# paLeziart/quadruped-reactive-walking

Hardware: AMD Instinct MI355X
Metric: control-steps/sec (MPC+WBC) (higher is better)
Workload: dtype f64

## Files before the change

### quadruped-reactive-walking_amd/csrc/chain_sweep.h

```cpp
#pragma once
#include <hip/hip_runtime.h>

#include "qrw_device.h"

namespace qrw {

constexpr int kCol = 14;
constexpr int kSlot = 168;
__host__ __device__ constexpr int chain_gap(int m) { return 0; }
__host__ __device__ constexpr int chain_slot(int slot, int m) { return slot * kSlot + (slot >= m ? chain_gap(m) : 0); }
__device__ __forceinline__ int chain_row_t(int lane) {
  const int l = lane & 15;
  return (l < 12) ? l : 11;
}
__host__ __device__ constexpr int chain_lds_doubles(int slots, int m) { return slots * kSlot + chain_gap(m); }

__device__ __forceinline__ double dpp_step12(double r, double x, const double (&m)[12]) {
  double a0 = r;
  asm("s_nop 1\n\t"
      "v_fmac_f64_dpp %0, %1, %2 row_newbcast:0 row_mask:0xf bank_mask:0xf\n\t"
      "v_fmac_f64_dpp %0, %1, %3 row_newbcast:1 row_mask:0xf bank_mask:0xf\n\t"
      "v_fmac_f64_dpp %0, %1, %4 row_newbcast:2 row_mask:0xf bank_mask:0xf\n\t"
      "v_fmac_f64_dpp %0, %1, %5 row_newbcast:3 row_mask:0xf bank_mask:0xf\n\t"
      "v_fmac_f64_dpp %0, %1, %6 row_newbcast:4 row_mask:0xf bank_mask:0xf\n\t"
// ... 28 lines not shown
  int lo = __double2loint(v), hi = __double2hiint(v);
  asm("s_nop 1\n\tv_permlane16_swap_b32 %0, %0\n\tv_permlane16_swap_b32 %1, %1" : "+v"(lo), "+v"(hi));
  return __hiloint2double(hi, lo);
}

template <int NC>
__device__ __forceinline__ void chain_forward_paired(const double* sN, double* sX, double* sDump, int lane) {
  constexpr int N = NC, m = N >> 1, LA = m, LB = N - 1 - m, NP = LA / 2;
  static_assert(LA % 2 == 0 && LB == LA - 1, "paired sweeps need an even chain length");
  const int i = ((lane & 15) < 12) ? (lane & 15) : 11;
  const int h = lane >> 5;
  const bool rw = (lane & 16) != 0;
  const bool own = (lane & 15) < 12;
  const double* pm = sN + (rw ? m * kSlot + chain_gap(m) : 0) + h * kSlot + i;
  double* px = sX + (rw ? (m + 1) * 12 : 0) + i;
  const double* pr = px + h * 12;
  double* dump = sDump + i;
  double* ps_odd = (own && h == 1) ? px : dump;
  double* ps_even = (own && h == 0) ? px : dump;
  double* ps_oddA = (own && h == 1 && !rw) ? px : dump;
  double x = px[0], pB = 0.0;
  ChainOp b0, b1;
  auto fetch = [&](ChainOp& b, int p) {
    const double* q = pm + 2 * p * kSlot;
#pragma unroll
    for (int c = 0; c < 12; c++) b.m[c] = __hip_atomic_load(q + c * kCol, __ATOMIC_RELAXED, __HIP_MEMORY_SCOPE_WAVEFRONT);
    b.r = pr[(2 * p + 1) * 12];
  };
  auto pair = [&](const ChainOp& b, int p) {
    const int t1 = 2 * p + 1, t2 = t1 + 1;
    x = dpp_step12(b.r, x, b.m);
    x = swap_halves(x);
    if (t1 == LB) pB = x;
    (t1 < LB ? ps_odd : ps_oddA)[t1 * 12] = x;
    x = dpp_step12(b.r, x, b.m);
    if (t2 < LA) {
      x = swap_halves(x);
      ps_even[t2 * 12] = x;
    }
  };
  fetch(b0, 0);
#pragma unroll
  for (int p = 0; p < NP; p += 2) {
    if (p + 1 < NP) fetch(b1, p + 1);
    __builtin_amdgcn_sched_barrier(0);
    pair(b0, p);
    if (p + 1 < NP) {
      if (p + 2 < NP) fetch(b0, p + 2);
      __builtin_amdgcn_sched_barrier(0);
      pair(b1, p + 1);
    }
  }
  x += swap_rows16(pB);
  if (lane >= 32 && lane < 44) sX[m * 12 + i] = x;
}
template <int NC>
__device__ __forceinline__ void chain_backward_paired(const double* sN, double* sX, double* sDump, int lane) {
  constexpr int N = NC, m = N >> 1, LA = m, LB = N - 1 - m, NP = LA / 2;
  static_assert(LA % 2 == 0 && LB == LA - 1, "paired sweeps need an even chain length");
  const int i = ((lane & 15) < 12) ? (lane & 15) : 11;
  const int h = lane >> 5;
  const bool rw = (lane & 16) != 0;
  const bool own = (lane & 15) < 12;
  const int ib = chain_row_t(lane);
  const double* pm = sN + ((rw ? (N - 1) : m) - LA - h) * kSlot + (rw ? chain_gap(m) : 0) + ib * kCol;
  double* px = sX + ((rw ? N : m) - LA) * 12 + i;
  const double* pr = px - h * 12;
  double* dump = sDump + i;
  double* ps_odd = (own && h == 1) ? px : dump;
  double* ps_even = (own && h == 0) ? px : dump;
  double* ps_lastA = (own && h == 1 && !rw) ? px : dump;
  double x = sX[m * 12 + i];
  ChainOp b0, b1;
  auto fetch = [&](ChainOp& b, int p) {
    const qrw_d2* q = reinterpret_cast<const qrw_d2*>(pm + (LA - 2 * p - 1) * kSlot);
#pragma unroll
    for (int c = 0; c < 6; c++) {
      const qrw_d2 v = q[c];
      b.m[2 * c] = v.x;
      b.m[2 * c + 1] = v.y;
    }
    b.r = pr[(LA - 2 * p - 1) * 12];
  };
  auto pair = [&](const ChainOp& b, int p) {
    const int t1 = 2 * p + 1, t2 = t1 + 1;
    x = dpp_step12(b.r, x, b.m);
    x = swap_halves(x);
    ps_odd[(LA - t1) * 12] = x;
    x = dpp_step12(b.r, x, b.m);
    if (t2 < LA) {
      x = swap_halves(x);
      ps_even[(LA - t2) * 12] = x;
    } else {
      ps_lastA[(LA - t2) * 12] = x;
    }
  };
  fetch(b0, 0);
#pragma unroll
  for (int p = 0; p < NP; p += 2) {
    if (p + 1 < NP) fetch(b1, p + 1);
    __builtin_amdgcn_sched_barrier(0);
    pair(b0, p);
    if (p + 1 < NP) {
      if (p + 2 < NP) fetch(b0, p + 2);
      __builtin_amdgcn_sched_barrier(0);
      pair(b1, p + 1);
    }
  }
}

template <int NC>
__device__ __forceinline__ void chain_forward_quad(const double* sN, double* sX, double* sDump, int lane) {
  constexpr int N = NC, m = N >> 1, LA = m, LB = N - 1 - m, NQ = LA / 4;
  static_assert(LA % 4 == 0 && LB == LA - 1, "the 2 + 2 half order needs a chain length that is a multiple of 4");
  const int i = ((lane & 15) < 12) ? (lane & 15) : 11;
  const int h = lane >> 5;
  const bool rw = (lane & 16) != 0;
  const bool own = (lane & 15) < 12;
  const double* pm = sN + (rw ? m * kSlot + chain_gap(m) : 0) + 2 * h * kSlot + i;
  double* px = sX + (rw ? (m + 1) * 12 : 0) + i;
  const double* pr = px + 2 * h * 12;
  double* dump = sDump + i;
  double* ps_lo = (own && h == 0) ? px : dump;
  double* ps_hi = (own && h == 1) ? px : dump;
  double* ps_hiA = (own && h == 1 && !rw) ? px : dump;
  double x = px[0], pB = 0.0;
  ChainOp bX, bY;
  auto fetch = [&](ChainOp& b, int s) {
    const double* q = pm + s * kSlot;
#pragma unroll
    for (int c = 0; c < 12; c++) b.m[c] = __hip_atomic_load(q + c * kCol, __ATOMIC_RELAXED, __HIP_MEMORY_SCOPE_WAVEFRONT);
    b.r = pr[(s + 1) * 12];
  };
  fetch(bX, 0);
  fetch(bY, 1);
#pragma unroll
  for (int q = 0; q < NQ; q++) {
    const int t = 4 * q;
    __builtin_amdgcn_sched_barrier(0);
    x = dpp_step12(bX.r, x, bX.m);
    ps_lo[(t + 1) * 12] = x;
    x = dpp_step12(bY.r, x, bY.m);
    x = swap_halves(x);
    ps_hi[(t + 2) * 12] = x;
    x = dpp_step12(bX.r, x, bX.m);
    if (t + 3 == LB) pB = x;
    (t + 3 < LB ? ps_hi : ps_hiA)[(t + 3) * 12] = x;
    if (q + 1 < NQ) fetch(bX, t + 4);
    __builtin_amdgcn_sched_barrier(0);
    x = dpp_step12(bY.r, x, bY.m);
    if (q + 1 < NQ) {
      x = swap_halves(x);
      ps_lo[(t + 4) * 12] = x;
      fetch(bY, t + 5);
    }
  }
  x += swap_rows16(pB);
  if (lane >= 32 && lane < 44) sX[m * 12 + i] = x;
}
template <int NC>
__device__ __forceinline__ void chain_backward_quad(const double* sN, double* sX, double* sDump, int lane) {
  constexpr int N = NC, m = N >> 1, LA = m, LB = N - 1 - m, NQ = LA / 4;
  static_assert(LA % 4 == 0 && LB == LA - 1, "the 2 + 2 half order needs a chain length that is a multiple of 4");
  const int i = ((lane & 15) < 12) ? (lane & 15) : 11;
  const int h = lane >> 5;
  const bool rw = (lane & 16) != 0;
  const bool own = (lane & 15) < 12;
  const int ib = chain_row_t(lane);
  const double* pm = sN + ((rw ? (N - 1) : m) - LA - 2 * h) * kSlot + (rw ? chain_gap(m) : 0) + ib * kCol;
  double* px = sX + ((rw ? N : m) - LA) * 12 + i;
  const double* pr = px - 2 * h * 12;
  double* dump = sDump + i;
  double* ps_lo = (own && h == 0) ? px : dump;
  double* ps_hi = (own && h == 1) ? px : dump;
  double* ps_lastA = (own && h == 1 && !rw) ? px : dump;
  double x = sX[m * 12 + i];
  ChainOp bX, bY;
  auto fetch = [&](ChainOp& b, int t) {
    const qrw_d2* q = reinterpret_cast<const qrw_d2*>(pm + (LA - t) * kSlot);
#pragma unroll
    for (int c = 0; c < 6; c++) {
      const qrw_d2 v = q[c];
      b.m[2 * c] = v.x;
      b.m[2 * c + 1] = v.y;
    }
    b.r = pr[(LA - t) * 12];
  };
  fetch(bX, 1);
  fetch(bY, 2);
#pragma unroll
  for (int q = 0; q < NQ; q++) {
    const int t = 4 * q;
    __builtin_amdgcn_sched_barrier(0);
    x = dpp_step12(bX.r, x, bX.m);
    ps_lo[(LA - t - 1) * 12] = x;
    x = dpp_step12(bY.r, x, bY.m);
    x = swap_halves(x);
    ps_hi[(LA - t - 2) * 12] = x;
    x = dpp_step12(bX.r, x, bX.m);
    ps_hi[(LA - t - 3) * 12] = x;
    if (q + 1 < NQ) fetch(bX, t + 5);
    __builtin_amdgcn_sched_barrier(0);
    x = dpp_step12(bY.r, x, bY.m);
    if (q + 1 < NQ) {
      x = swap_halves(x);
      ps_lo[(LA - t - 4) * 12] = x;
      fetch(bY, t + 6);
    } else {
      ps_lastA[0] = x;
    }
  }
// ... 154 lines not shown
```

### quadruped-reactive-walking_amd/csrc/mpc_kernel.hip

```cpp
#include <hip/hip_runtime.h>
#include <math.h>
#include <stdint.h>

#include <type_traits>
#include <vector>

#include "chain_sweep.h"
#include "qrw_device.h"
#include "qrw_kernels.h"

namespace qrw {

namespace {

constexpr int kMatSz = 144;
constexpr int kWSz = 36;

template <int NW>
struct alignas(16) MpcLdsT {
  static constexpr int S = 16 * NW;
  double sN[chain_lds_doubles(S, S / 2)];
  double sX[(S + 2) * 12];
  double sDump[(S / 2 + 2) * 12];
  double sE[S * 12];
  double sW[S * kWSz];
  double sOm[S * 12];
  double sDg[S * 12];
  double sA[kMatSz];
  double sB[kMatSz];
  double sRed[4];
  unsigned long long sBal[2];
  double sPre[8];
};

template <int NW>
__device__ __forceinline__ void wg_sync_t() {
  if constexpr (NW == 1) asm volatile("" ::: "memory");
  else __syncthreads();
}
#define wg_sync() wg_sync_t<NW>()
#ifdef QRW_PROFILE_PHASES
#define PH_DECL unsigned long long ph_t0 = __builtin_amdgcn_s_memtime(), ph_acc[10] = {0,0,0,0,0,0,0,0,0,0};
#ifndef QRW_PH_MASK
#define QRW_PH_MASK 0x3FF
#endif
#define PH(i) do { if ((QRW_PH_MASK >> (i)) & 1) { unsigned long long t_ = __builtin_amdgcn_s_memtime(); ph_acc[i] += t_ - ph_t0; ph_t0 = t_; } } while (0)
#elif defined(QRW_MARK_PHASES)
#define PH_DECL
#define PH(i) asm volatile("; QRW_PHASE " #i)
#else
#define PH_DECL
#define PH(i)
#endif

__device__ __forceinline__ void cone_apply(const double f[3], double mu, double out[5]) {
  out[0] = f[0] - mu * f[2];
  out[1] = -f[0] - mu * f[2];
  out[2] = f[1] - mu * f[2];
  out[3] = -f[1] - mu * f[2];
  out[4] = -f[2];
}
__device__ __forceinline__ void cone_apply_t(const double w[5], double mu, double out[3]) {
  out[0] = w[0] - w[1];
  out[1] = w[2] - w[3];
  out[2] = -mu * (w[0] + w[1] + w[2] + w[3]) - w[4];
}

template <int NW, bool CL = false>
__device__ __forceinline__ void nb_next(const double v[3], double same[3], double shifted[3], double* sE, int k, int j,
                                        int lane, bool has_next) {
  if constexpr (NW == 1) {
    const int s4 = (CL && !has_next) ? lane : lane + 4, s2 = (CL && !has_next) ? lane : lane + 2;
#pragma unroll
    for (int t = 0; t < 3; t++) { same[t] = shfl(v[t], s4); shifted[t] = shfl(v[t], s2); }
  } else {
#pragma unroll
    for (int t = 0; t < 3; t++) sE[k * 12 + 3 * j + t] = v[t];
    __syncthreads();
    const int kn = has_next ? k + 1 : k;
#pragma unroll
    for (int t = 0; t < 3; t++) { same[t] = sE[kn * 12 + 3 * j + t]; shifted[t] = sE[kn * 12 + 3 * ((j + 2) & 3) + t]; }
    __syncthreads();
  }
}
template <int NW, bool CL = false>
__device__ __forceinline__ void nb_prev(const double v[3], double same[3], double shifted[3], double* sE, int k, int j,
                                        int lane, bool has_prev) {
  if constexpr (NW == 1) {
    const int s4 = (CL && !has_prev) ? lane : lane - 4, s2 = (CL && !has_prev) ? lane : lane - 2;
#pragma unroll
    for (int t = 0; t < 3; t++) { same[t] = shfl(v[t], s4); shifted[t] = shfl(v[t], s2); }
  } else {
#pragma unroll
// ... 374 lines not shown
  return task;
}
template <int NW>
__device__ __forceinline__ bool pre_may_park(const MpcArgs& a, unsigned long long* sh, int tid) {
  int ok = 0;
  if (tid == 0) ok = pre_claim(a) ? 1 : 0;
  if constexpr (NW == 1) {
    ok = __builtin_amdgcn_readfirstlane(ok);
  } else {
    int* si = reinterpret_cast<int*>(sh);
    __syncthreads();
    if (tid == 0) si[0] = ok;
    __syncthreads();
    ok = si[0];
    __syncthreads();
  }
  return ok != 0;
}
__device__ __forceinline__ int pre_level(const MpcArgs& a, int iter, int it_resume, double r, double r_prev) {
  if (a.pre_levels < 2 || it_resume == 0) return 0;
  const int nl = a.pre_levels - 1;
  float rem = (float)(4000 - iter);
  if (r_prev > r && r > 1.0) rem = fminf(rem, 200.0f * __logf((float)r) / __logf((float)(r_prev / r)));
  int bin = (int)(rem / (float)a.pre_bin);
  bin = bin < 0 ? 0 : (bin > nl - 1 ? nl - 1 : bin);
  return 1 + (nl - 1 - bin);
}
template <int NW>
__device__ __forceinline__ void pre_end_chunk(const MpcArgs& a, int b, bool parked, int level, int tid) {
  asm volatile("s_waitcnt vmcnt(0)" ::: "memory");
  if constexpr (NW > 1) __syncthreads();
  if (tid == 0) {
    if (parked) {
      __builtin_amdgcn_fence(__ATOMIC_RELEASE, "agent");
      asm volatile("s_waitcnt vmcnt(0)" ::: "memory");
      const unsigned slot = __hip_atomic_fetch_add(&a.pre_ctr[kPreLevelWord + 2 * level + 1], 1u, __ATOMIC_RELAXED, __HIP_MEMORY_SCOPE_AGENT);
      if (slot < (unsigned)a.pre_cap) __hip_atomic_store(&a.pre_queue[(size_t)level * a.pre_cap + slot], b, __ATOMIC_RELAXED, __HIP_MEMORY_SCOPE_AGENT);
      else pre_set_error(a, 2u);
      __hip_atomic_fetch_add(&a.pre_ctr[kPreParks], 1u, __ATOMIC_RELAXED, __HIP_MEMORY_SCOPE_AGENT);
    } else {
      __hip_atomic_fetch_add(&a.pre_ctr[kPreDone], 1u, __ATOMIC_RELAXED, __HIP_MEMORY_SCOPE_AGENT);
    }
    __hip_atomic_fetch_add(&a.pre_ctr[kPreProgress], 1u, __ATOMIC_RELAXED, __HIP_MEMORY_SCOPE_AGENT);
  }
}

template <int NW, bool FULL, bool SEQ, bool PRE = false>
__global__ __launch_bounds__(64 * NW, 1) void mpc_solve_kernel(MpcArgs a) {
  static_assert(!(SEQ && PRE), "one queueing mode at a time");
  __shared__ MpcLdsT<NW> L;
  constexpr int T = 64 * NW;
  PH_DECL
  const int tid = threadIdx.x;
  const int lane = tid & 63, wv = tid >> 6;
#ifdef QRW_DEBUG_POISON
  if constexpr (!SEQ && !PRE) {
    const double qnan = __longlong_as_double(-1ll);
    auto fill = [&](double* p, int n) { for (int e = tid; e < n; e += 64 * NW) p[e] = qnan; };
    switch (a.pre_bin) {
      case 1: fill(L.sN, (int)(sizeof(L.sN) / 8)); break;
      case 2: fill(L.sX, (int)(sizeof(L.sX) / 8)); break;
      case 3: fill(L.sDump, (int)(sizeof(L.sDump) / 8)); break;
      case 4: fill(L.sE, (int)(sizeof(L.sE) / 8)); break;
      case 5: fill(L.sW, (int)(sizeof(L.sW) / 8)); break;
      case 6: fill(L.sOm, (int)(sizeof(L.sOm) / 8)); break;
      case 7: fill(L.sDg, (int)(sizeof(L.sDg) / 8)); break;
      case 8: fill(L.sA, kMatSz); break;
      case 9: fill(L.sB, kMatSz); break;
      case 10: fill(L.sRed, 4); fill(L.sPre, 8); break;
      default: break;
    }
    __syncthreads();
  }
#endif
  {
  int b, seq_s = 0;
#ifdef QRW_SEQ_STATS
  unsigned long long task_t0 = 0;
#endif
  if constexpr (SEQ) {
    const int task = seq_next_task<NW>(a, &L.sBal[0], tid, (int)blockIdx.x < a.seq_groups);
    if (task < 0) return;
#ifdef QRW_SEQ_STATS
    task_t0 = __builtin_amdgcn_s_memrealtime();
#endif
    seq_s = task / a.B;
    b = task - seq_s * a.B;
  } else if constexpr (PRE) {
    if ((int)blockIdx.x + a.pre_block0 < a.B) {
      b = a.order ? a.order[blockIdx.x] : blockIdx.x;
    } else {
      b = pre_next_task<NW>(a, &L.sBal[0], tid);
      if (b < 0) return;
    }
  } else {
    b = a.order ? a.order[blockIdx.x] : blockIdx.x;
  }
  int it_resume = 0;
  bool aborted = false;
  if constexpr (PRE) {
    const int pit = __hip_atomic_load(&a.pause_it[b], __ATOMIC_RELAXED, __HIP_MEMORY_SCOPE_AGENT);
    if ((int)blockIdx.x + a.pre_block0 >= a.B) it_resume = pit;
    else aborted = (pit != 0);
  }
  const bool resumed = PRE && it_resume > 0;
  if constexpr (PRE) { if (tid < 8) L.sPre[tid] = 0.0; }
#ifdef QRW_TRACE_RES
  if (!resumed && a.prof) for (int e = tid; e < kMpcProfItems; e += T) a.prof[(size_t)b * kMpcProfItems + e] = 0.0;
#endif
  const int k = 16 * wv + (lane >> 2), j = lane & 3;
  const int N = a.N;
  const bool act = FULL ? true : (k < N);
  const bool has_next = act && (k + 1 < N);
  const bool has_prev = act && (k > 0);
  const bool next_here = has_next;
  const double mN = next_here ? 1.0 : 0.0, mN6 = (next_here && j >= 2) ? a.dt : 0.0;
  const double mP = has_prev ? 1.0 : 0.0, mP6 = (has_prev && j < 2) ? a.dt : 0.0;
  const double mG = (j >= 2) ? 1.0 : 0.0, mGN = (j >= 2 && next_here) ? 1.0 : 0.0;
  const int kp = has_prev ? k - 1 : k;
  const int kx = act ? chain_pos(k, N >> 1, N) : k;
  const int kpx = act ? chain_pos(kp, N >> 1, N) : k;
  if (tid < 24) L.sX[N * 12 + tid] = 0.0;
  for (int e = tid; e < kSlot; e += T) L.sN[chain_slot(16 * NW - 1, N >> 1) + e] = 0.0;

  const double dt = a.dt;
  const double mass = (double)2.50000279f;
  const double mu = (double)0.9f;
  const double dtm = dt / mass;
  const double g8 = (double)(9.81f) * dt;
  const double wF = (double)5e-5f;
  const double sigma = 1e-6, alpha = 1.6;
  const double eps_abs = 1e-6, eps_rel = 1e-6;
  const double w_all[12] = {2.0, 2.0, 20.0, 0.25, 0.25, 10.0, (double)0.2f, (double)0.2f,
                            (double)0.2f, 0.0, 0.0, (double)0.3f};
  double wX[3];
#pragma unroll
  for (int t = 0; t < 3; t++) wX[t] = (j == 0) ? w_all[t] : (j == 1) ? w_all[3 + t] : (j == 2) ? w_all[6 + t] : w_all[9 + t];

  const size_t io = (size_t)seq_s * a.B + b;
  const double* xr = a.xref + io * 12 * (N + 1);
  const double* fs = a.fsteps + io * a.N_gait * 12;
  double* outp = a.out + io * 24 * N;
  double* st = a.st + (size_t)b * kMpcStItems * T;
  const int num_iter = (a.num_iter ? a.num_iter[b] : a.num_iter_scalar) + seq_s;
  const bool first = (num_iter == 0);
  bool parked = false;
#define ST(item) st[(item)*T + tid]

  if (!first && !__hip_atomic_load(&a.flags[b], __ATOMIC_RELAXED, __HIP_MEMORY_SCOPE_AGENT)) {
    if (tid == 0) {
// ... 218 lines not shown
    nC[4] = Ec[4] * Df0[2];
    double colsum = 0.0;
#pragma unroll
    for (int t = 0; t < 3; t++) {
      Dx0[t] *= rsqrt(limit_scaling(nX[t]));
      Df0[t] *= rsqrt(limit_scaling(nF[t]));
      Ed[t] *= rsqrt(limit_scaling(nD[t]));
      Es[t] *= rsqrt(limit_scaling(nS[t]));
      colsum += fabs(cs * wX[t] * Dx0[t] * Dx0[t]) + fabs(cs * wF * Df0[t] * Df0[t]);
    }
#pragma unroll
    for (int c = 0; c < 5; c++) Ec[c] *= rsqrt(limit_scaling(nC[c]));
    double ct = block_sum<NW>(act ? colsum : 0.0, L.sRed, wv, lane) * inv_n;
    ct = fmax(ct, 1.0);
    ct = limit_scaling(ct);
    cs *= 1.0 / ct;
  }
  const double cinv = 1.0 / cs;
  double iDx[3], iDf[3];
#pragma unroll
  for (int t = 0; t < 3; t++) { iDx[t] = 1.0 / Dx0[t]; iDf[t] = 1.0 / Df0[t]; }
  double xhX[3], xhF[3], thD[3], etS[3], zeC[5], etC[5];
#pragma unroll
  for (int t = 0; t < 3; t++) {
    xhX[t] = resumed ? xX[t] : Dx0[t] * xX[t];
    xhF[t] = resumed ? xF[t] : Df0[t] * xF[t];
    etS[t] = resumed ? yS[t] : Es[t] * yS[t];
  }
#pragma unroll
  for (int c = 0; c < 5; c++) etC[c] = resumed ? yC[c] : Ec[c] * yC[c];
  double aOD[3], kD[3], zeU[3], aOS[3], aOC[5], sDx2[3], sDf2[3], lz4 = 0.0;
#pragma unroll
  for (int t = 0; t < 3; t++) {
    aOD[t] = kD[t] = zeU[t] = aOS[t] = thD[t] = 0.0;
    sDx2[t] = sigma * iDx[t] * iDx[t]; sDf2[t] = sigma * iDf[t] * iDf[t];
  }
#pragma unroll
  for (int c = 0; c < 5; c++) aOC[c] = zeC[c] = 0.0;
  const double aVel = (j >= 2) ? alpha : 0.0;
  double wD[3];
  double wnV[3] = {0.0, 0.0, 0.0}, wn6V[3] = {0.0, 0.0, 0.0};
  double rho_used = 1.0;

  double Dinv[6], Kr[2][6];
  AccD Di[3][12];
#pragma unroll
  for (int t = 0; t < 3; t++)
#pragma unroll
    for (int c = 0; c < 12; c++) Di[t][c].set(0.0);
#pragma unroll
  for (int c = 0; c < 6; c++) Dinv[c] = Kr[0][c] = Kr[1][c] = 0.0;
  const int kr1 = (j < 2) ? j + 4 : j;

  bool need_factor = true;
  int iter = 0, status = kStatusUnsolved, rho_updates = 0;
  double pri_res = 0.0, dua_res = 0.0, last_np = 0.0, last_nd = 0.0;
  const int max_iter = 4000;
  rho = fmin(fmax(rho, kRhoMin), kRhoMax);
  {
    rho_used = resumed ? ST(kStC) : rho;
    const double rho_eq0 = kRhoEqOverIneq * rho_used;
#pragma unroll
    for (int t = 0; t < 3; t++) {
      zeU[t] = (rho_eq0 * Ed[t] * Ed[t]) * uD0[t];
      const double eta = Ed[t] * yD[t], ze0 = rho_eq0 * Ed[t] * zD[t];
      const double th0 = (eta + (1.0 - alpha) * (ze0 - zeU[t])) - zeU[t];
      thD[t] = resumed ? yD[t] : th0;
      wD[t] = act ? (resumed ? -yD[t] : ze0 - eta) : 0.0;
    }
#pragma unroll
    for (int c = 0; c < 5; c++) zeC[c] = resumed ? zC[c] : rho * Ec[c] * zC[c];
    if (resumed) rho_updates = __hip_atomic_load(&a.rho_updates[b], __ATOMIC_RELAXED, __HIP_MEMORY_SCOPE_AGENT);
  }
  bool same_rho_resume = resumed && (rho == rho_used);
  AccD pEd[3], pEs[3], pEc[5], pIDx[3], pIDf[3], pUD0[3], pWX[3], pCs;
#pragma unroll
  for (int t = 0; t < 3; t++) {
    pEd[t].set(Ed[t]); pEs[t].set(Es[t]); pIDx[t].set(iDx[t]); pIDf[t].set(iDf[t]); pUD0[t].set(uD0[t]); pWX[t].set(wX[t]);
  }
#pragma unroll
  for (int c = 0; c < 5; c++) pEc[c].set(Ec[c]);
  pCs.set(cs);
#define QRW_UNPARK()                                                                                        \
  double Ed[3], Es[3], Ec[5], iDx[3], iDf[3], uD0[3], wX[3];                                                \
  _Pragma("unroll") for (int t = 0; t < 3; t++) {                                                           \
    Ed[t] = pEd[t].get(); Es[t] = pEs[t].get(); iDx[t] = pIDx[t].get(); iDf[t] = pIDf[t].get();              \
    uD0[t] = pUD0[t].get(); wX[t] = pWX[t].get();                                                           \
  }                                                                                                         \
  _Pragma("unroll") for (int c = 0; c < 5; c++) Ec[c] = pEc[c].get();                                       \
  const double cs = pCs.get();

  PH(8);
  for (iter = it_resume + 1; iter <= max_iter; iter++) {
    PH(9);
    if (need_factor) {
      need_factor = false;
      QRW_UNPARK()
      const double rho_eq = kRhoEqOverIneq * rho;
      double omD[3], omS[3], omC[5];
#pragma unroll
      for (int t = 0; t < 3; t++) { omD[t] = rho_eq * Ed[t] * Ed[t]; omS[t] = rho_eq * Es[t] * Es[t]; }
#pragma unroll
      for (int c = 0; c < 5; c++) omC[c] = rho * Ec[c] * Ec[c];
      {
#pragma unroll
        for (int t = 0; t < 3; t++) {
          const double zu_new = omD[t] * uD0[t];
          double shift = zu_new - zeU[t];
          if constexpr (PRE) shift = same_rho_resume ? 0.0 : shift;
          thD[t] -= shift;
          wD[t] = act ? wD[t] + shift : 0.0;
          zeU[t] = zu_new;
          aOD[t] = (j >= 2) ? 0.0 : alpha * omD[t];
          kD[t] = alpha * zu_new;
          aOS[t] = alpha * omS[t] * sfl[t];
        }
        const double rs = rho / rho_used;
#pragma unroll
        for (int c = 0; c < 5; c++) {
          zeC[c] *= rs;
          aOC[c] = alpha * omC[c];
        }
        rho_used = rho;
        same_rho_resume = false;
        lz4 = omC[4] * -25.0;
      }
      double omL[3], omA[3], Kinv[6][6];
#pragma unroll
      for (int t = 0; t < 3; t++) { omL[t] = quad_bcast<2>(omD[t]); omA[t] = quad_bcast<3>(omD[t]); }
      force_block_factor(act, Bang, sfl, iDf, omL, omA, omS, omC, cs, wF, sigma, dtm, mu, Dinv, Kinv);
      wg_sync();
      if (act) {
        if (j == 0) {
#pragma unroll
          for (int c = 0; c < 6; c++)
#pragma unroll
            for (int c2 = 0; c2 < 6; c2++) L.sW[k * kWSz + c * 6 + c2] = Kinv[c][c2];
        }
#pragma unroll
        for (int t = 0; t < 3; t++) {
          L.sOm[k * 12 + 3 * j + t] = omD[t];
          L.sDg[k * 12 + 3 * j + t] = cs * wX[t] + sigma * iDx[t] * iDx[t];
        }
      }
      wg_sync();
#pragma unroll
      for (int c = 0; c < 6; c++) { Kr[0][c] = L.sW[k * kWSz + j * 6 + c]; Kr[1][c] = L.sW[k * kWSz + kr1 * 6 + c]; }
      {
        double DiV[3][12];
#pragma unroll
        for (int t = 0; t < 3; t++)
#pragma unroll
          for (int c = 0; c < 12; c++) DiV[t][c] = Di[t][c].get();
        chain_factorize<T>(L, N, dt, tid, k, j, DiV);
#pragma unroll
        for (int t = 0; t < 3; t++)
#pragma unroll
          for (int c = 0; c < 12; c++) Di[t][c].set(DiV[t][c]);
      }
      nb_next<NW, !FULL>(wD, wnV, wn6V, L.sE, k, j, lane, has_next);
    PH(0);
    }

    double wC[5];
#pragma unroll
    for (int c = 0; c < 5; c++) wC[c] = zeC[c] - etC[c];
    double rX[3], rF[3], coneT[3];
    cone_apply_t(wC, mu, coneT);
#pragma unroll
    for (int t = 0; t < 3; t++) {
      const double wn = wnV[t], wn6 = wn6V[t];
      const double v = mN * wn + mN6 * wn6 - wD[t];
      rX[t] = sDx2[t] * xhX[t] + v;
    }
    {
      double wL[3], wA[3];
#pragma unroll
      for (int t = 0; t < 3; t++) { wL[t] = quad_bcast<2>(wD[t]); wA[t] = quad_bcast<3>(wD[t]); }
#pragma unroll
      for (int t = 0; t < 3; t++) {
        double v = dtm * wL[t] - sfl[t] * etS[t] + coneT[t];
#pragma unroll
        for (int r = 0; r < 3; r++) v += Bang[r][t] * wA[r];
        rF[t] = sDf2[t] * xhF[t] + v;
      }
    }
    PH(1);
    double tF[3], yK[6];
    {
      tF[0] = Dinv[0] * rF[0] + Dinv[1] * rF[1] + Dinv[2] * rF[2];
      tF[1] = Dinv[1] * rF[0] + Dinv[3] * rF[1] + Dinv[4] * rF[2];
      tF[2] = Dinv[2] * rF[0] + Dinv[4] * rF[1] + Dinv[5] * rF[2];
      double sK[6];
#pragma unroll
      for (int t = 0; t < 3; t++) {
        sK[t] = dtm * quad_sum(act ? tF[t] : 0.0);
        sK[3 + t] = quad_sum(act ? Bang[t][0] * tF[0] + Bang[t][1] * tF[1] + Bang[t][2] * tF[2] : 0.0);
      }
      kinv_apply(Kr, sK, yK);
      double gsV[3], gnV[3], gdum[3];
#pragma unroll
      for (int t = 0; t < 3; t++) gsV[t] = -((j == 3) ? yK[3 + t] : yK[t]);
      nb_next<NW, !FULL>(gsV, gnV, gdum, L.sE, k, j, lane, has_next);
#pragma unroll
      for (int t = 0; t < 3; t++) rX[t] += mGN * gnV[t] - mG * gsV[t];
    }
    PH(2);
    {
      if (act) {
#pragma unroll
        for (int t = 0; t < 3; t++) L.sX[kx * 12 + 3 * j + t] = rX[t];
      }
      wg_sync();
      if (wv == 0) chain_forward<FULL ? 16 * NW : 0>(L.sN, L.sX, L.sDump, N, lane);
      wg_sync();
      PH(3);
// ... 20 lines not shown
      if (wv == 0) chain_backward<FULL ? 16 * NW : 0>(L.sN, L.sX, L.sDump, N, lane);
      wg_sync();
      PH(5);
    }
    double dV[6], fh[3], xh[3], xpi[3], xpi6[3], dK[6];
    {
      const double* xc = &L.sX[kx * 12];
      const double* xp = &L.sX[kpx * 12];
#pragma unroll
      for (int c = 0; c < 6; c++) dV[c] = xc[6 + c] - mP * xp[6 + c];
#pragma unroll
      for (int t = 0; t < 3; t++) {
        xh[t] = xc[3 * j + t];
        xpi[t] = xp[3 * j + t];
        xpi6[t] = xp[3 * ((j + 2) & 3) + t];
      }
      double wB[3];
      kinv_apply(Kr, dV, dK);
#pragma unroll
      for (int c = 0; c < 6; c++) dK[c] = yK[c] - dK[c];
#pragma unroll
      for (int t = 0; t < 3; t++) wB[t] = dtm * dK[t] + Bang[0][t] * dK[3] + Bang[1][t] * dK[4] + Bang[2][t] * dK[5];
      fh[0] = tF[0] - (Dinv[0] * wB[0] + Dinv[1] * wB[1] + Dinv[2] * wB[2]);
      fh[1] = tF[1] - (Dinv[1] * wB[0] + Dinv[3] * wB[1] + Dinv[4] * wB[2]);
      fh[2] = tF[2] - (Dinv[2] * wB[0] + Dinv[4] * wB[1] + Dinv[5] * wB[2]);
#pragma unroll
      for (int t = 0; t < 3; t++) fh[t] = act ? fh[t] : 0.0;
    }
    {
      double cv[5];
      cone_apply(fh, mu, cv);
#pragma unroll
      for (int t = 0; t < 3; t++) {
        const double v = mP * xpi[t] + mP6 * xpi6[t] - xh[t];
        const double dsel = (j == 3) ? dK[3 + t] : dK[t];
        xhX[t] = alpha * xh[t] + (1.0 - alpha) * xhX[t];
        xhF[t] = alpha * fh[t] + (1.0 - alpha) * xhF[t];
        thD[t] = fma(aVel, dsel, fma(aOD[t], v, thD[t])) - kD[t];
        wD[t] = act ? -thD[t] : 0.0;
        etS[t] = fma(aOS[t], fh[t], etS[t]);
      }
      nb_next<NW, !FULL>(wD, wnV, wn6V, L.sE, k, j, lane, has_next);
#pragma unroll
      for (int c = 0; c < 5; c++) {
        const double s_ = fma(aOC[c], cv[c], (1.0 - alpha) * zeC[c]) + etC[c];
        double zn = (c == 4) ? fmax(s_, lz4) : s_;
        zn = fmin(zn, 0.0);
        etC[c] = s_ - zn;
        zeC[c] = zn;
      }
    }

    PH(6);
    const bool check = (iter % 25 == 0);
    if (check) {
      PH(6);
      QRW_UNPARK()
      const double cinv = fast_rcp(cs);
      double Dx[3], Df[3], iEd[3], iEs[3], iEc[5];
#pragma unroll
      for (int t = 0; t < 3; t++) { Dx[t] = fast_rcp(iDx[t]); Df[t] = fast_rcp(iDf[t]); iEd[t] = fast_rcp(Ed[t]); iEs[t] = fast_rcp(Es[t]); }
#pragma unroll
      for (int c = 0; c < 5; c++) iEc[c] = fast_rcp(Ec[c]);
      double zD[3], zC[5];
#pragma unroll
      for (int t = 0; t < 3; t++) zD[t] = Ed[t] * uD0[t];
#pragma unroll
      for (int c = 0; c < 5; c++) zC[c] = zeC[c] * (iEc[c] * fast_rcp(rho_used));
      wg_sync();
      if (act) {
#pragma unroll
        for (int t = 0; t < 3; t++) L.sX[kx * 12 + 3 * j + t] = xhX[t];
      }
      wg_sync();
      double pres = 0.0, nz = 0.0, nax = 0.0, pres_s = 0.0, nz_s = 0.0, nax_s = 0.0;
      {
        double pl[3], pa[3];
#pragma unroll
        for (int t = 0; t < 3; t++) {
          pl[t] = quad_sum(act ? xhF[t] : 0.0);
          pa[t] = quad_sum(act ? Bang[t][0] * xhF[0] + Bang[t][1] * xhF[1] + Bang[t][2] * xhF[2] : 0.0);
        }
#pragma unroll
        for (int t = 0; t < 3; t++) {
          const int i = 3 * j + t;
          double v = -xhX[t];
          if (has_prev) {
            v += L.sX[kpx * 12 + i];
            if (j < 2) v += dt * L.sX[kpx * 12 + i + 6];
          }
          if (j == 2) v += dtm * pl[t];
          if (j == 3) v += pa[t];
          const double axs = Ed[t] * v;
          const double rs = axs - zD[t];
          pres_s = fmax(pres_s, fabs(rs)); nz_s = fmax(nz_s, fabs(zD[t])); nax_s = fmax(nax_s, fabs(axs));
          pres = fmax(pres, fabs(iEd[t] * rs)); nz = fmax(nz, fabs(iEd[t] * zD[t])); nax = fmax(nax, fabs(iEd[t] * axs));
          const double axS = Es[t] * sfl[t] * xhF[t];
          pres_s = fmax(pres_s, fabs(axS)); nax_s = fmax(nax_s, fabs(axS));
          pres = fmax(pres, fabs(iEs[t] * axS)); nax = fmax(nax, fabs(iEs[t] * axS));
        }
        double cv[5];
        cone_apply(xhF, mu, cv);
#pragma unroll
        for (int c = 0; c < 5; c++) {
          const double axs = Ec[c] * cv[c];
          const double rs = axs - zC[c];
          pres_s = fmax(pres_s, fabs(rs)); nz_s = fmax(nz_s, fabs(zC[c])); nax_s = fmax(nax_s, fabs(axs));
          pres = fmax(pres, fabs(iEc[c] * rs)); nz = fmax(nz, fabs(iEc[c] * zC[c])); nax = fmax(nax, fabs(iEc[c] * axs));
        }
      }
      if (!act) { pres = nz = nax = 0.0; pres_s = nz_s = nax_s = 0.0; }
      pres = block_max<NW>(pres, L.sRed, wv, lane); nz = block_max<NW>(nz, L.sRed, wv, lane);
      nax = block_max<NW>(nax, L.sRed, wv, lane);
      pri_res = pres;
#ifdef QRW_TRACE_RES
      if (tid == 0 && a.prof) a.prof[(size_t)b * kMpcProfItems + 64 + (iter / 25 - 1)] = pres / (eps_abs + eps_rel * fmax(nz, nax));
#endif
      last_np = fmax(nz, nax);
      const bool pri_ok = pri_res < eps_abs + eps_rel * last_np;
      const bool need_dual = pri_ok || (iter % 200 == 0) || (iter == max_iter) || (pri_res > kOsqpInfty);
      double dres = 0.0, naty = 0.0, npx = 0.0, dres_s = 0.0, naty_s = 0.0, npx_s = 0.0;
      if (need_dual) {
        double eD[3], eS[3], eC[5], cT[3];
#pragma unroll
        for (int t = 0; t < 3; t++) { eD[t] = act ? thD[t] + zeU[t] : 0.0; eS[t] = etS[t]; }
#pragma unroll
        for (int c = 0; c < 5; c++) eC[c] = etC[c];
        cone_apply_t(eC, mu, cT);
        double eL[3], eA[3];
#pragma unroll
        for (int t = 0; t < 3; t++) { eL[t] = quad_bcast<2>(eD[t]); eA[t] = quad_bcast<3>(eD[t]); }
        double enV[3], en6V[3];
        nb_next<NW, !FULL>(eD, enV, en6V, L.sE, k, j, lane, has_next);
#pragma unroll
        for (int t = 0; t < 3; t++) {
          const double en = enV[t], en6 = en6V[t];
          double aty = -eD[t];
          if (has_next) {
            aty += en;
            if (j >= 2) aty += dt * en6;
          }
          const double px = cs * wX[t] * xhX[t];
          dres = fmax(dres, fabs(px + aty)); naty = fmax(naty, fabs(aty)); npx = fmax(npx, fabs(px));
          dres_s = fmax(dres_s, fabs(Dx[t] * (px + aty))); naty_s = fmax(naty_s, fabs(Dx[t] * aty));
          npx_s = fmax(npx_s, fabs(Dx[t] * px));
          double atf = dtm * eL[t] + sfl[t] * eS[t] + cT[t];
#pragma unroll
          for (int r = 0; r < 3; r++) atf += Bang[r][t] * eA[r];
          const double pf = cs * wF * xhF[t];
          dres = fmax(dres, fabs(pf + atf)); naty = fmax(naty, fabs(atf)); npx = fmax(npx, fabs(pf));
          dres_s = fmax(dres_s, fabs(Df[t] * (pf + atf))); naty_s = fmax(naty_s, fabs(Df[t] * atf));
          npx_s = fmax(npx_s, fabs(Df[t] * pf));
        }
        if (!act) { dres = naty = npx = 0.0; dres_s = naty_s = npx_s = 0.0; }
        dres = block_max<NW>(dres, L.sRed, wv, lane); naty = block_max<NW>(naty, L.sRed, wv, lane);
        npx = block_max<NW>(npx, L.sRed, wv, lane);
        dua_res = cinv * dres;
        last_nd = cinv * fmax(naty, npx);
      }
      bool done = false;
      if (need_dual) {
        if (pri_res > kOsqpInfty || dua_res > kOsqpInfty) {
          status = kStatusNonCvx;
          done = true;
        } else if (pri_ok && dua_res < eps_abs + eps_rel * last_nd) {
          status = kStatusSolved;
          done = true;
        }
      }
      if (done) break;
      if (iter % 200 == 0) {
        pres_s = block_max<NW>(pres_s, L.sRed, wv, lane); nz_s = block_max<NW>(nz_s, L.sRed, wv, lane);
        nax_s = block_max<NW>(nax_s, L.sRed, wv, lane); dres_s = block_max<NW>(dres_s, L.sRed, wv, lane);
        naty_s = block_max<NW>(naty_s, L.sRed, wv, lane); npx_s = block_max<NW>(npx_s, L.sRed, wv, lane);
        const double pn = pres_s / (fmax(nz_s, nax_s) + 1e-10);
        const double dn = dres_s / (fmax(naty_s, npx_s) + 1e-10);
        double rho_new = rho * sqrt(pn / (dn + 1e-10));
        rho_new = fmin(fmax(rho_new, kRhoMin), kRhoMax);
        if (rho_new > rho * 5.0 || rho_new < rho / 5.0) {
          rho = rho_new;
          rho_updates++;
          need_factor = true;
        }
#ifdef QRW_TRACE_RES
        if (tid == 0 && a.prof && iter <= 4000) {
          double* tr = a.prof + (size_t)b * kMpcProfItems + (iter / 200 - 1) * 3;
          tr[0] = pri_res / (eps_abs + eps_rel * last_np); tr[1] = dua_res / (eps_abs + eps_rel * last_nd); tr[2] = rho;
        }
#endif
        if constexpr (PRE) {
          if (iter - it_resume >= a.pre_chunk && iter < max_iter) {
            if (pre_may_park<NW>(a, &L.sBal[0], tid)) parked = true;
            else it_resume = iter;
          }
          if (tid == 0) {
            double* pr = &L.sPre[(iter / 200 & 1) * 4];
            pr[0] = pri_res; pr[1] = last_np; pr[2] = dua_res; pr[3] = last_nd;
          }
        }
      }
      PH(7);
      if constexpr (PRE) {
        if (parked) break;
      }
    }
  }
  PH(7);
#ifdef QRW_PROFILE_PHASES
  if (tid == 0 && a.prof) for (int i = 0; i < 10; i++) a.prof[(size_t)b * kMpcProfItems + i] = (double)ph_acc[i];
#endif
  if (iter > max_iter) iter = max_iter;
  if (status == kStatusUnsolved && !parked) {
    const bool pok = pri_res < 10.0 * eps_abs + 10.0 * eps_rel * last_np;
    const bool dok = dua_res < 10.0 * eps_abs + 10.0 * eps_rel * last_nd;
    status = (pok && dok) ? kStatusSolvedInaccurate : kStatusMaxIter;
  }

  {
  QRW_UNPARK()
  const bool has_sol = (status != kStatusNonCvx);
  if (act && !parked) {
#pragma unroll
    for (int t = 0; t < 3; t++) {
      const int i = 3 * j + t;
      const double sx = has_sol ? xhX[t] + xr[i * (N + 1) + k + 1] : nan("");
      const double sf = has_sol ? xhF[t] : nan("");
      outp[i * N + k] = sx;
      outp[(12 + i) * N + k] = sf;
    }
  }
#pragma unroll
  for (int t = 0; t < 3; t++) {
    xX[t] = parked ? xhX[t] : xhX[t] * iDx[t]; xF[t] = parked ? xhF[t] : xhF[t] * iDf[t];
    zD[t] = Ed[t] * uD0[t];
    yD[t] = parked ? thD[t] : (thD[t] + zeU[t]) * (1.0 / Ed[t]);
    yS[t] = parked ? etS[t] : etS[t] * (1.0 / Es[t]);
  }
#pragma unroll
  for (int c = 0; c < 5; c++) {
    zC[c] = parked ? zeC[c] : zeC[c] * (1.0 / (rho_used * Ec[c]));
    yC[c] = parked ? etC[c] : etC[c] * (1.0 / Ec[c]);
  }
  if (!has_sol) {
#pragma unroll
    for (int t = 0; t < 3; t++) xX[t] = xF[t] = zD[t] = yD[t] = yS[t] = 0.0;
#pragma unroll
    for (int c = 0; c < 5; c++) zC[c] = yC[c] = 0.0;
  }
  ST(kStRho) = rho;
  ST(kStC) = parked ? rho_used : cs;
#pragma unroll
  for (int t = 0; t < 3; t++) {
    ST(kStXX + t) = xX[t]; ST(kStXF + t) = xF[t]; ST(kStZD + t) = zD[t];
    ST(kStYD + t) = yD[t]; ST(kStYS + t) = yS[t]; ST(kStS + t) = sfl[t];
    ST(kStDX + t) = 1.0 / iDx[t]; ST(kStDF + t) = 1.0 / iDf[t]; ST(kStED + t) = Ed[t]; ST(kStES + t) = Es[t];
#pragma unroll
    for (int r = 0; r < 3; r++) ST(kStB + r * 3 + t) = Bang[r][t];
  }
#pragma unroll
  for (int c = 0; c < 5; c++) { ST(kStZC + c) = zC[c]; ST(kStYC + c) = yC[c]; ST(kStEC + c) = Ec[c]; }
  if (PRE && parked) {
    if (tid == 0) {
      a.pause_it[b] = iter;
      a.rho_updates[b] = rho_updates;
    }
  } else if (tid == 0) {
    if constexpr (PRE) a.pause_it[b] = 0;
    a.flags[b] = 1;
    a.iters[b] = iter;
    a.status[b] = status;
    a.rho_out[b] = rho;
    a.pri[b] = pri_res;
    a.dua[b] = dua_res;
    a.rho_updates[b] = rho_updates;
    if (SEQ && a.seq_iters) a.seq_iters[io] = iter;
#ifdef QRW_SEQ_STATS
    if (a.prof && a.seq_K <= 5) {
      a.prof[io * 2] = (double)(__builtin_amdgcn_s_memrealtime() - task_t0);
      a.prof[io * 2 + 1] = (double)iter;
    }
#endif
  }
  }
  }
  if constexpr (SEQ) seq_finish_task<NW>(a, b, seq_s, tid);
  if constexpr (PRE) {
    int level = 0;
    if (parked && tid == 0) {
      const int it = a.pause_it[b];
      const double* p1 = &L.sPre[(it / 200 & 1) * 4];
      const double* p0 = &L.sPre[((it / 200 & 1) ^ 1) * 4];
      const double r1 = fmax(p1[0] / (1e-6 + 1e-6 * p1[1]), p1[2] / (1e-6 + 1e-6 * p1[3]));
      const double r0 = (p0[1] > 0.0 || p0[3] > 0.0) ? fmax(p0[0] / (1e-6 + 1e-6 * p0[1]), p0[2] / (1e-6 + 1e-6 * p0[3])) : 0.0;
      level = pre_level(a, it, it_resume, r1, r0);
    }
    pre_end_chunk<NW>(a, b, parked, level, tid);
  }
  }
#undef QRW_UNPARK
#undef ST
}

namespace {
__device__ __forceinline__ int order_key(float e) {
  const int key = (int)(e * 0.04f);
  return key < 0 ? 0 : (key > 160 ? 160 : key);
}
__device__ __forceinline__ float order_ema(float e0, float it) { return (e0 == 0.0f) ? it : e0 + (it - e0) * 0.125f; }
}

__global__ __launch_bounds__(64) void mpc_order_kernel(const int* __restrict__ iters, float* __restrict__ ema,
                                                       int* __restrict__ order, int B) {
  constexpr int U = 4, R = 64 * 4 * U;
  __shared__ int hist[162];
  __shared__ int offs[162];
  const int lane = threadIdx.x;
  for (int i = lane; i < 162; i += 64) hist[i] = 0;
  __syncthreads();
  const int Bv = B - B % R;
  for (int base = 0; base < Bv; base += R) {
    int4 it[U];
    float4 e[U];
#pragma unroll
    for (int u = 0; u < U; u++) {
      const int b = base + (u * 64 + lane) * 4;
      it[u] = *reinterpret_cast<const int4*>(iters + b);
      e[u] = *reinterpret_cast<const float4*>(ema + b);
    }
#pragma unroll
    for (int u = 0; u < U; u++) {
      const int b = base + (u * 64 + lane) * 4;
      e[u].x = order_ema(e[u].x, (float)it[u].x);
      e[u].y = order_ema(e[u].y, (float)it[u].y);
      e[u].z = order_ema(e[u].z, (float)it[u].z);
      e[u].w = order_ema(e[u].w, (float)it[u].w);
      *reinterpret_cast<float4*>(ema + b) = e[u];
      atomicAdd(&hist[order_key(e[u].x)], 1);
      atomicAdd(&hist[order_key(e[u].y)], 1);
      atomicAdd(&hist[order_key(e[u].z)], 1);
      atomicAdd(&hist[order_key(e[u].w)], 1);
    }
  }
  for (int b = Bv + lane; b < B; b += 64) {
    const float e = order_ema(ema[b], (float)iters[b]);
    ema[b] = e;
    atomicAdd(&hist[order_key(e)], 1);
  }
  __syncthreads();
  {
    const int k0 = 160 - 3 * lane;
    int h[3], tot = 0;
#pragma unroll
    for (int j = 0; j < 3; j++) { h[j] = (k0 - j >= 0) ? hist[k0 - j] : 0; tot += h[j]; }
    int incl = tot;
#pragma unroll
    for (int d = 1; d < 64; d <<= 1) {
      const int up = __shfl_up(incl, d, 64);
      if (lane >= d) incl += up;
    }
    int run = incl - tot;
#pragma unroll
    for (int j = 0; j < 3; j++) { if (k0 - j >= 0) offs[k0 - j] = run; run += h[j]; }
  }
  __syncthreads();
  for (int base = 0; base < Bv; base += R) {
    float4 e[U];
#pragma unroll
    for (int u = 0; u < U; u++) e[u] = *reinterpret_cast<const float4*>(ema + base + (u * 64 + lane) * 4);
#pragma unroll
    for (int u = 0; u < U; u++) {
      const int b = base + (u * 64 + lane) * 4;
      order[atomicAdd(&offs[order_key(e[u].x)], 1)] = b;
      order[atomicAdd(&offs[order_key(e[u].y)], 1)] = b + 1;
      order[atomicAdd(&offs[order_key(e[u].z)], 1)] = b + 2;
      order[atomicAdd(&offs[order_key(e[u].w)], 1)] = b + 3;
    }
  }
  for (int b = Bv + lane; b < B; b += 64) order[atomicAdd(&offs[order_key(ema[b])], 1)] = b;
}

int mpc_order_launch(const int* iters, float* ema, int* order, int B, hipStream_t stream) {
  hipLaunchKernelGGL(mpc_order_kernel, dim3(1), dim3(64), 0, stream, iters, ema, order, B);
  return hipGetLastError() == hipSuccess ? 0 : -2;
}

int mpc_preemptive_launch(const MpcArgs& a_in, int resident_slots, hipStream_t stream) {
  if (a_in.N <= 16 || a_in.N > kMpcMaxN || !a_in.pre_queue || !a_in.pre_ctr || !a_in.pause_it || a_in.pre_chunk < 200 || a_in.pre_cmax < 1 ||
      a_in.pre_levels < 1 || a_in.pre_levels > kPreMaxLevels || a_in.pre_bin < 1) return -1;
  MpcArgs a = a_in;
  auto go = [&](unsigned blocks) {
    if (a.N == 32) hipLaunchKernelGGL((mpc_solve_kernel<2, true, false, true>), dim3(blocks), dim3(128), 0, stream, a);
    else hipLaunchKernelGGL((mpc_solve_kernel<2, false, false, true>), dim3(blocks), dim3(128), 0, stream, a);
  };
  const unsigned takers = (unsigned)a.B * (unsigned)(a.pre_cmax - 1);
  if (a.B > resident_slots || takers == 0u) {
    a.pre_block0 = 0;
    go((unsigned)a.B + takers);
  } else {
    a.pre_block0 = 0;
    go((unsigned)a.B);
    a.pre_block0 = a.B;
    go(takers);
  }
  return hipGetLastError() == hipSuccess ? 0 : -2;
}

__global__ void mpc_pre_error_flush_kernel(const unsigned* pre_ctr, unsigned* host_word) {
  const unsigned code = pre_ctr[kPreErr];
  if (code != 0u) __hip_atomic_store(host_word, code, __ATOMIC_RELAXED, __HIP_MEMORY_SCOPE_SYSTEM);
}
int mpc_pre_error_flush(const unsigned* pre_ctr, unsigned* host_word, hipStream_t stream) {
  hipLaunchKernelGGL(mpc_pre_error_flush_kernel, dim3(1), dim3(1), 0, stream, pre_ctr, host_word);
  return hipGetLastError() == hipSuccess ? 0 : -2;
}

int mpc_launch(const MpcArgs& a, hipStream_t stream) {
  if (a.N < 1 || a.N > kMpcMaxN) return -1;
  if (a.N == 16) hipLaunchKernelGGL((mpc_solve_kernel<1, true, false>), dim3(a.B), dim3(64), 0, stream, a);
  else if (a.N < 16) hipLaunchKernelGGL((mpc_solve_kernel<1, false, false>), dim3(a.B), dim3(64), 0, stream, a);
  else if (a.N == 32) hipLaunchKernelGGL((mpc_solve_kernel<2, true, false>), dim3(a.B), dim3(128), 0, stream, a);
  else hipLaunchKernelGGL((mpc_solve_kernel<2, false, false>), dim3(a.B), dim3(128), 0, stream, a);
  return hipGetLastError() == hipSuccess ? 0 : -2;
}

__global__ void mpc_seq_init_kernel(int* queue, unsigned* qctr, int* level, int* first, const int* order, int B, int K, int groups) {
  __shared__ unsigned n_lvl[kSeqLevels], base[kSeqLevels], n_q[kSeqLevels], n_dealt[kSeqLevels];
  const int cut[kSeqLevels] = {B / 16, B / 4, B / 2, B};
  auto level_of = [&](int rank) {
    if (!order) return kSeqLevels - 1;
    for (int l = 0; l < kSeqLevels; l++) if (rank < cut[l]) return l;
    return kSeqLevels - 1;
  };
  if (threadIdx.x == 0) {
    unsigned run = 0;
    for (int l = 0; l < kSeqLevels; l++) {
      const int lo = (l == 0) ? 0 : cut[l - 1];
      n_lvl[l] = order ? (unsigned)(cut[l] - lo) : (l == kSeqLevels - 1 ? (unsigned)B : 0u);
      base[l] = run;
      run += n_lvl[l] * (unsigned)K;
      n_q[l] = 0;
// ... 145 lines not shown
```

Before: 701,500.

## Restructure ADMM loop into fixed check intervals and cut register pressure

```diff
diff --git a/quadruped-reactive-walking_amd/csrc/chain_sweep.h b/quadruped-reactive-walking_amd/csrc/chain_sweep.h
--- a/quadruped-reactive-walking_amd/csrc/chain_sweep.h
+++ b/quadruped-reactive-walking_amd/csrc/chain_sweep.h
@@ -104,7 +104,7 @@
     }
   }
   x += swap_rows16(pB);
-  if (lane >= 32 && lane < 44) sX[m * 12 + i] = x;
+  ps_oddA[m * 12] = x;
 }
 template <int NC>
 __device__ __forceinline__ void chain_backward_paired(const double* sN, double* sX, double* sDump, int lane) {
@@ -208,7 +208,7 @@
     }
   }
   x += swap_rows16(pB);
-  if (lane >= 32 && lane < 44) sX[m * 12 + i] = x;
+  ps_hiA[m * 12] = x;
 }
 template <int NC>
 __device__ __forceinline__ void chain_backward_quad(const double* sN, double* sX, double* sDump, int lane) {
diff --git a/quadruped-reactive-walking_amd/csrc/mpc_kernel.hip b/quadruped-reactive-walking_amd/csrc/mpc_kernel.hip
--- a/quadruped-reactive-walking_amd/csrc/mpc_kernel.hip
+++ b/quadruped-reactive-walking_amd/csrc/mpc_kernel.hip
@@ -39,6 +39,11 @@
   else __syncthreads();
 }
 #define wg_sync() wg_sync_t<NW>()
+
+__device__ __forceinline__ bool uniform_flag(bool c) { return __builtin_amdgcn_readfirstlane((int)c) != 0; }
+__device__ __forceinline__ double uniform_double(double v) {
+  return __hiloint2double(__builtin_amdgcn_readfirstlane(__double2hiint(v)), __builtin_amdgcn_readfirstlane(__double2loint(v)));
+}
 #ifdef QRW_PROFILE_PHASES
 #define PH_DECL unsigned long long ph_t0 = __builtin_amdgcn_s_memtime(), ph_acc[10] = {0,0,0,0,0,0,0,0,0,0};
 #ifndef QRW_PH_MASK
@@ -519,7 +524,7 @@
   constexpr int T = 64 * NW;
   PH_DECL
   const int tid = threadIdx.x;
-  const int lane = tid & 63, wv = tid >> 6;
+  const int lane = tid & 63, wv = (NW == 1) ? 0 : tid >> 6;
 #ifdef QRW_DEBUG_POISON
   if constexpr (!SEQ && !PRE) {
     const double qnan = __longlong_as_double(-1ll);
@@ -563,6 +568,10 @@
   } else {
     b = a.order ? a.order[blockIdx.x] : blockIdx.x;
   }
+  if constexpr (SEQ || PRE) {
+    b = __builtin_amdgcn_readfirstlane(b);
+    seq_s = __builtin_amdgcn_readfirstlane(seq_s);
+  }
   int it_resume = 0;
   bool aborted = false;
   if constexpr (PRE) {
@@ -887,13 +896,15 @@
   for (int c = 0; c < 6; c++) Dinv[c] = Kr[0][c] = Kr[1][c] = 0.0;
   const int kr1 = (j < 2) ? j + 4 : j;
 
-  bool need_factor = true;
+  int need_factor_entry = 1;
+  asm volatile("" : "+s"(need_factor_entry));
+  bool need_factor = need_factor_entry != 0;
   int iter = 0, status = kStatusUnsolved, rho_updates = 0;
   double pri_res = 0.0, dua_res = 0.0, last_np = 0.0, last_nd = 0.0;
   const int max_iter = 4000;
-  rho = fmin(fmax(rho, kRhoMin), kRhoMax);
+  rho = uniform_double(fmin(fmax(rho, kRhoMin), kRhoMax));
   {
-    rho_used = resumed ? ST(kStC) : rho;
+    rho_used = uniform_double(resumed ? ST(kStC) : rho);
     const double rho_eq0 = kRhoEqOverIneq * rho_used;
 #pragma unroll
     for (int t = 0; t < 3; t++) {
@@ -908,29 +919,43 @@
     if (resumed) rho_updates = __hip_atomic_load(&a.rho_updates[b], __ATOMIC_RELAXED, __HIP_MEMORY_SCOPE_AGENT);
   }
   bool same_rho_resume = resumed && (rho == rho_used);
-  AccD pEd[3], pEs[3], pEc[5], pIDx[3], pIDf[3], pUD0[3], pWX[3], pCs;
+  AccD pEd[3], pEs[3], pEc[5], pIDx[3], pIDf[3], pUD0[3], pCs;
+  AccD pNp, pDua, pNd;
+  pNp.set(0.0); pDua.set(0.0); pNd.set(0.0);
 #pragma unroll
   for (int t = 0; t < 3; t++) {
-    pEd[t].set(Ed[t]); pEs[t].set(Es[t]); pIDx[t].set(iDx[t]); pIDf[t].set(iDf[t]); pUD0[t].set(uD0[t]); pWX[t].set(wX[t]);
+    pEd[t].set(Ed[t]); pEs[t].set(Es[t]); pIDx[t].set(iDx[t]); pIDf[t].set(iDf[t]); pUD0[t].set(uD0[t]);
   }
 #pragma unroll
   for (int c = 0; c < 5; c++) pEc[c].set(Ec[c]);
   pCs.set(cs);
-#define QRW_UNPARK()                                                                                        \
+#define QRW_UNPARK()                                                                                         \
   double Ed[3], Es[3], Ec[5], iDx[3], iDf[3], uD0[3], wX[3];                                                \
   _Pragma("unroll") for (int t = 0; t < 3; t++) {                                                           \
     Ed[t] = pEd[t].get(); Es[t] = pEs[t].get(); iDx[t] = pIDx[t].get(); iDf[t] = pIDf[t].get();              \
-    uD0[t] = pUD0[t].get(); wX[t] = pWX[t].get();                                                           \
+    uD0[t] = pUD0[t].get();                                                                                   \
   }                                                                                                         \
   _Pragma("unroll") for (int c = 0; c < 5; c++) Ec[c] = pEc[c].get();                                       \
-  const double cs = pCs.get();
+  const double cs = pCs.get();                                                                              \
+  _Pragma("unroll") for (int t = 0; t < 3; t++)                                                             \
+    wX[t] = (j == 0) ? w_all[t] : (j == 1) ? w_all[3 + t] : (j == 2) ? w_all[6 + t] : w_all[9 + t];
+#define QRW_ZETA_U()                                                                                        \
+  double zeU[3];                                                                                            \
+  _Pragma("unroll") for (int t = 0; t < 3; t++) {                                                           \
+    zeU[t] = ((kRhoEqOverIneq * rho_used) * Ed[t] * Ed[t]) * uD0[t];                                        \
+    asm volatile("" : "+v"(zeU[t]));                                                                        \
+  }
 
   PH(8);
-  for (iter = it_resume + 1; iter <= max_iter; iter++) {
+  constexpr int kCheckEvery = 25;
+  static_assert(max_iter % kCheckEvery == 0 && 200 % kCheckEvery == 0, "checks, rho tests and max_iter fall on interval ends");
+  iter = it_resume;
+  for (;;) {
     PH(9);
     if (need_factor) {
       need_factor = false;
       QRW_UNPARK()
+      QRW_ZETA_U()
       const double rho_eq = kRhoEqOverIneq * rho;
       double omD[3], omS[3], omC[5];
 #pragma unroll
@@ -945,7 +970,6 @@
           if constexpr (PRE) shift = same_rho_resume ? 0.0 : shift;
           thD[t] -= shift;
           wD[t] = act ? wD[t] + shift : 0.0;
-          zeU[t] = zu_new;
           aOD[t] = (j >= 2) ? 0.0 : alpha * omD[t];
           kD[t] = alpha * zu_new;
           aOS[t] = alpha * omS[t] * sfl[t];
@@ -997,6 +1021,8 @@
     PH(0);
     }
 
+#pragma nounroll
+    for (int plain = 0; plain < kCheckEvery; plain++) {
     double wC[5];
 #pragma unroll
     for (int c = 0; c < 5; c++) wC[c] = zeC[c] - etC[c];
@@ -1123,10 +1149,11 @@
     }
 
     PH(6);
-    const bool check = (iter % 25 == 0);
-    if (check) {
-      PH(6);
+    }
+    iter += kCheckEvery;
+    {
       QRW_UNPARK()
+      QRW_ZETA_U()
       const double cinv = fast_rcp(cs);
       double Dx[3], Df[3], iEd[3], iEs[3], iEc[5];
 #pragma unroll
@@ -1183,14 +1210,16 @@
       if (!act) { pres = nz = nax = 0.0; pres_s = nz_s = nax_s = 0.0; }
       pres = block_max<NW>(pres, L.sRed, wv, lane); nz = block_max<NW>(nz, L.sRed, wv, lane);
       nax = block_max<NW>(nax, L.sRed, wv, lane);
-      pri_res = pres;
+      pri_res = uniform_double(pres);
 #ifdef QRW_TRACE_RES
       if (tid == 0 && a.prof) a.prof[(size_t)b * kMpcProfItems + 64 + (iter / 25 - 1)] = pres / (eps_abs + eps_rel * fmax(nz, nax));
 #endif
       last_np = fmax(nz, nax);
+      pNp.set(last_np);
       const bool pri_ok = pri_res < eps_abs + eps_rel * last_np;
-      const bool need_dual = pri_ok || (iter % 200 == 0) || (iter == max_iter) || (pri_res > kOsqpInfty);
+      const bool need_dual = uniform_flag(pri_ok || pri_res > kOsqpInfty) || (iter % 200 == 0) || (iter == max_iter);
       double dres = 0.0, naty = 0.0, npx = 0.0, dres_s = 0.0, naty_s = 0.0, npx_s = 0.0;
+      dua_res = last_nd = 0.0;
       if (need_dual) {
         double eD[3], eS[3], eC[5], cT[3];
 #pragma unroll
@@ -1228,18 +1257,18 @@
         npx = block_max<NW>(npx, L.sRed, wv, lane);
         dua_res = cinv * dres;
         last_nd = cinv * fmax(naty, npx);
-      }
-      bool done = false;
+        pDua.set(dua_res); pNd.set(last_nd);
+      }
       if (need_dual) {
-        if (pri_res > kOsqpInfty || dua_res > kOsqpInfty) {
+        if (uniform_flag(pri_res > kOsqpInfty || dua_res > kOsqpInfty)) {
           status = kStatusNonCvx;
-          done = true;
-        } else if (pri_ok && dua_res < eps_abs + eps_rel * last_nd) {
+          break;
+        }
+        if (uniform_flag(pri_ok && dua_res < eps_abs + eps_rel * last_nd)) {
           status = kStatusSolved;
-          done = true;
-        }
-      }
-      if (done) break;
+          break;
+        }
+      }
       if (iter % 200 == 0) {
         pres_s = block_max<NW>(pres_s, L.sRed, wv, lane); nz_s = block_max<NW>(nz_s, L.sRed, wv, lane);
         nax_s = block_max<NW>(nax_s, L.sRed, wv, lane); dres_s = block_max<NW>(dres_s, L.sRed, wv, lane);
@@ -1248,8 +1277,8 @@
         const double dn = dres_s / (fmax(naty_s, npx_s) + 1e-10);
         double rho_new = rho * sqrt(pn / (dn + 1e-10));
         rho_new = fmin(fmax(rho_new, kRhoMin), kRhoMax);
-        if (rho_new > rho * 5.0 || rho_new < rho / 5.0) {
-          rho = rho_new;
+        if (uniform_flag(rho_new > rho * 5.0 || rho_new < rho / 5.0)) {
+          rho = uniform_double(rho_new);
           rho_updates++;
           need_factor = true;
         }
@@ -1261,7 +1290,7 @@
 #endif
         if constexpr (PRE) {
           if (iter - it_resume >= a.pre_chunk && iter < max_iter) {
-            if (pre_may_park<NW>(a, &L.sBal[0], tid)) parked = true;
+            if (uniform_flag(pre_may_park<NW>(a, &L.sBal[0], tid))) parked = true;
             else it_resume = iter;
           }
           if (tid == 0) {
@@ -1275,12 +1304,14 @@
         if (parked) break;
       }
     }
+    if (iter >= max_iter) break;
   }
   PH(7);
 #ifdef QRW_PROFILE_PHASES
   if (tid == 0 && a.prof) for (int i = 0; i < 10; i++) a.prof[(size_t)b * kMpcProfItems + i] = (double)ph_acc[i];
 #endif
   if (iter > max_iter) iter = max_iter;
+  last_np = pNp.get(); dua_res = pDua.get(); last_nd = pNd.get();
   if (status == kStatusUnsolved && !parked) {
     const bool pok = pri_res < 10.0 * eps_abs + 10.0 * eps_rel * last_np;
     const bool dok = dua_res < 10.0 * eps_abs + 10.0 * eps_rel * last_nd;
@@ -1288,7 +1319,11 @@
   }
 
   {
+  int tid_e = threadIdx.x;
+  asm volatile("" : "+v"(tid_e));
+  const int tid = tid_e, k = 16 * ((NW == 1) ? 0 : tid_e >> 6) + ((tid_e & 63) >> 2), j = tid_e & 3;
   QRW_UNPARK()
+  QRW_ZETA_U()
   const bool has_sol = (status != kStatusNonCvx);
   if (act && !parked) {
 #pragma unroll
@@ -1369,6 +1404,7 @@
   }
   }
 #undef QRW_UNPARK
+#undef QRW_ZETA_U
 #undef ST
 }
 
@@ -1456,7 +1492,7 @@
 }
 
 int mpc_preemptive_launch(const MpcArgs& a_in, int resident_slots, hipStream_t stream) {
-  if (a_in.N <= 16 || a_in.N > kMpcMaxN || !a_in.pre_queue || !a_in.pre_ctr || !a_in.pause_it || a_in.pre_chunk < 200 || a_in.pre_cmax < 1 ||
+  if (a_in.N <= 16 || a_in.N > kMpcMaxN || !a_in.pre_queue || !a_in.pre_ctr || !a_in.pause_it || a_in.pre_chunk < 200 || a_in.pre_chunk % 200 != 0 || a_in.pre_cmax < 1 ||
       a_in.pre_levels < 1 || a_in.pre_levels > kPreMaxLevels || a_in.pre_bin < 1) return -1;
   MpcArgs a = a_in;
   auto go = [&](unsigned blocks) {
```

Measured after the change: 750,500 (median of 6 runs). 7.0% higher.
